# constantinpape/torch-em

Hardware: AMD Instinct MI355X
Metric: voxels/sec fwd+bwd, UNet3d 1x128^3 bs=2 (higher is better)
Workload: dtype f32-class (forward convs on normalised activations: fp32 operands split into 2 fp16 terms = 22 mantissa bits, lo plane scaled by 2^12 with its own fp32 accumulator, 3 fp16 MFMAs per product; other forward convs 3 bf16 terms / 6 MFMAs; data-gradient convs 2 bf16 terms / 3 MFMAs (16-bit products); WEI

## Files before the change

torch_em_amd/csrc/capi.hip:

```cpp
#include "tem_common.h"
#include "conv_internal.h"
#include "tem_act.h"
#include <stdarg.h>
#include <string.h>

static thread_local char g_err[512] = "";

void tem_set_error(const char* fmt, ...) {
    va_list ap;
    va_start(ap, fmt);
    vsnprintf(g_err, sizeof(g_err), fmt, ap);
    va_end(ap);
}

extern "C" const char* tem_last_error(void) { return g_err; }

struct TemOption {
    const char* name;
    long long def;
};
static const TemOption g_opt_table[TEM_OPT_COUNT] = {
    {"wgrad_zs", 3},
    {"wgrad_zs_persist", 1},
    {"wgrad_sums", 1},
    {"wgrad_sums_min_mb", 128},
    {"fwd_persistent", -1},
    {"conv_fwd_variant", -1},
    {"conv1x1_stream", 1},
    {"fwd_ksplit_chunks", 0},
    {"wgrad_cus", 256},
    {"upsample_generic", 0},
    {"team_min_units", 0},
    {"zr_splitk", 1},
    {"zr_wide", 1},
    {"zr_tile_blocks", 1},
    {"dice_vox", 1},
    {"upsample2_ch8", 1},
    {"pool_vec8", 2},
    {"fp32_zr", 1},
};
static long long g_opt_val[TEM_OPT_COUNT];
static bool g_opt_set[TEM_OPT_COUNT];

long long tem_option(int id) {
    if (id < 0 || id >= TEM_OPT_COUNT) return 0;
    return __atomic_load_n(&g_opt_set[id], __ATOMIC_RELAXED) ? __atomic_load_n(&g_opt_val[id], __ATOMIC_RELAXED)
                                                            : g_opt_table[id].def;
}
static int opt_find(const char* name) {
    if (!name) return -1;
    for (int i = 0; i < TEM_OPT_COUNT; ++i)
        if (!strcmp(name, g_opt_table[i].name)) return i;
    return -1;
}
extern "C" int tem_set_option(const char* name, int64_t value) {
    const int id = opt_find(name);
    TEM_REQUIRE(id >= 0, "tem_set_option: unknown option '%s'", name ? name : "(null)");
    __atomic_store_n(&g_opt_val[id], (long long)value, __ATOMIC_RELAXED);
    __atomic_store_n(&g_opt_set[id], true, __ATOMIC_RELAXED);
    return TEM_OK;
}
extern "C" int tem_get_option(const char* name, int64_t* value) {
    const int id = opt_find(name);
    TEM_REQUIRE(id >= 0 && value, "tem_get_option: unknown option '%s'", name ? name : "(null)");
    *value = (int64_t)tem_option(id);
    return TEM_OK;
}
extern "C" int tem_version(void) { return 100; }

extern "C" int tem_device_cus(void) {
    int dev = 0;
    if (hipGetDevice(&dev) != hipSuccess) return TEM_ELAUNCH;
    hipDeviceProp_t prop;
    if (hipGetDeviceProperties(&prop, dev) != hipSuccess) return TEM_ELAUNCH;
    return prop.multiProcessorCount;
}

#define TT_V 64
#define TT_C 32

__global__ __launch_bounds__(256) void k_nchw_to_nhwc(const float* __restrict__ src, float* __restrict__ dst,
                                                      int64_t dst_ld, int C, int64_t V, int64_t vtiles, int ctiles) {
    __shared__ float tile[TT_C][TT_V + 1];
    int64_t ntiles = vtiles * ctiles;
    int n = blockIdx.y;
    for (int64_t t = blockIdx.x; t < ntiles; t += gridDim.x) {
        int ct = (int)(t % ctiles);
        int64_t vt = t / ctiles;
        int64_t v0 = vt * TT_V;
        int c0 = ct * TT_C;
        for (int i = threadIdx.x; i < TT_C * TT_V; i += 256) {
            int c = i / TT_V, v = i % TT_V;
            float val = 0.f;
            if (c0 + c < C && v0 + v < V) val = src[((int64_t)n * C + c0 + c) * V + v0 + v];
            tile[c][v] = val;
        }
        __syncthreads();
        for (int i = threadIdx.x; i < TT_C * TT_V; i += 256) {
            int v = i / TT_C, c = i % TT_C;
            if (c0 + c < C && v0 + v < V) dst[((int64_t)n * V + v0 + v) * dst_ld + c0 + c] = tile[c][v];
        }
        __syncthreads();
    }
}

__global__ __launch_bounds__(256) void k_nhwc_to_nchw(const float* __restrict__ src, int64_t src_ld,
                                                      float* __restrict__ dst, int C, int64_t V, int64_t vtiles,
                                                      int ctiles) {
    __shared__ float tile[TT_C][TT_V + 1];
    int64_t ntiles = vtiles * ctiles;
    int n = blockIdx.y;
    for (int64_t t = blockIdx.x; t < ntiles; t += gridDim.x) {
        int ct = (int)(t % ctiles);
        int64_t vt = t / ctiles;
        int64_t v0 = vt * TT_V;
        int c0 = ct * TT_C;
        for (int i = threadIdx.x; i < TT_C * TT_V; i += 256) {
            int v = i / TT_C, c = i % TT_C;
            float val = 0.f;
            if (c0 + c < C && v0 + v < V) val = src[((int64_t)n * V + v0 + v) * src_ld + c0 + c];
            tile[c][v] = val;
        }
        __syncthreads();
        for (int i = threadIdx.x; i < TT_C * TT_V; i += 256) {
            int c = i / TT_V, v = i % TT_V;
            if (c0 + c < C && v0 + v < V) dst[((int64_t)n * C + c0 + c) * V + v0 + v] = tile[c][v];
        }
        __syncthreads();
    }
}

extern "C" int tem_nchw_to_nhwc(const float* src, float* dst, int64_t dst_ld, int N, int C, int64_t V,
                                tem_stream_t stream) {
    TEM_REQUIRE(src && dst && N > 0 && C > 0 && V > 0 && dst_ld >= C, "tem_nchw_to_nhwc: bad arguments");
    int64_t vtiles = tem_cdiv(V, TT_V);
    int ctiles = (int)tem_cdiv(C, TT_C);
    int64_t nt = vtiles * ctiles;
    dim3 grid((unsigned)(nt > 4096 ? 4096 : nt), N);
    hipLaunchKernelGGL(k_nchw_to_nhwc, grid, dim3(256), 0, (hipStream_t)stream, src, dst, dst_ld, C, V, vtiles, ctiles);
    TEM_CHECK_LAUNCH("tem_nchw_to_nhwc");
    return TEM_OK;
}

extern "C" int tem_nhwc_to_nchw(const float* src, int64_t src_ld, float* dst, int N, int C, int64_t V,
                                tem_stream_t stream) {
    TEM_REQUIRE(src && dst && N > 0 && C > 0 && V > 0 && src_ld >= C, "tem_nhwc_to_nchw: bad arguments");
    int64_t vtiles = tem_cdiv(V, TT_V);
    int ctiles = (int)tem_cdiv(C, TT_C);
    int64_t nt = vtiles * ctiles;
    dim3 grid((unsigned)(nt > 4096 ? 4096 : nt), N);
    hipLaunchKernelGGL(k_nhwc_to_nchw, grid, dim3(256), 0, (hipStream_t)stream, src, src_ld, dst, C, V, vtiles, ctiles);
    TEM_CHECK_LAUNCH("tem_nhwc_to_nchw");
    return TEM_OK;
}

#define STD_BLOCKS 256

__global__ __launch_bounds__(256) void k_std_partial(const float* __restrict__ x, int64_t L, double* __restrict__ part) {
    int n = blockIdx.y;
    const float* row = x + (int64_t)n * L;
    double s = 0.0, ss = 0.0;
    for (int64_t i = (int64_t)blockIdx.x * 256 + threadIdx.x; i < L; i += (int64_t)gridDim.x * 256) {
        double v = (double)row[i];
        s += v;
        ss += v * v;
    }
    s = tem_wave_sum_d(s);
    ss = tem_wave_sum_d(ss);
    __shared__ double sh[2][4];
    int w = threadIdx.x >> 6;
    if ((threadIdx.x & 63) == 0) { sh[0][w] = s; sh[1][w] = ss; }
    __syncthreads();
    if (threadIdx.x == 0) {
        part[((int64_t)n * gridDim.x + blockIdx.x) * 2 + 0] = sh[0][0] + sh[0][1] + sh[0][2] + sh[0][3];
        part[((int64_t)n * gridDim.x + blockIdx.x) * 2 + 1] = sh[1][0] + sh[1][1] + sh[1][2] + sh[1][3];
    }
}

__global__ __launch_bounds__(256) void k_std_apply(const float* __restrict__ x, float* __restrict__ y, int64_t L,
                                                   const double* __restrict__ part, int nblk, float eps) {
    int n = blockIdx.y;
    __shared__ float sh_mean, sh_inv;
    if (threadIdx.x == 0) {
        double s = 0.0, ss = 0.0;
        for (int b = 0; b < nblk; ++b) {
            s += part[((int64_t)n * nblk + b) * 2 + 0];
            ss += part[((int64_t)n * nblk + b) * 2 + 1];
        }
        double mean = s / (double)L;
        double var = ss / (double)L - mean * mean;
        if (var < 0.0) var = 0.0;
        sh_mean = (float)mean;
        sh_inv = (float)(1.0 / (sqrt(var) + (double)eps));
    }
    __syncthreads();
    float mean = sh_mean, inv = sh_inv;
    const float* row = x + (int64_t)n * L;
    float* out = y + (int64_t)n * L;
    for (int64_t i = (int64_t)blockIdx.x * 256 + threadIdx.x; i < L; i += (int64_t)gridDim.x * 256)
        out[i] = (row[i] - mean) * inv;
}

extern "C" int tem_standardize(const float* x, float* y, int N, int64_t L, float eps, void* ws, int64_t ws_bytes,
                               tem_stream_t stream) {
    TEM_REQUIRE(x && y && ws && N > 0 && L > 0, "tem_standardize: bad arguments");
    int nblk = (int)(tem_cdiv(L, 256) < STD_BLOCKS ? tem_cdiv(L, 256) : STD_BLOCKS);
    if ((int64_t)N * nblk * 2 * (int64_t)sizeof(double) > ws_bytes) {
        tem_set_error("tem_standardize: workspace too small (%lld bytes needed)",
                      (long long)((int64_t)N * nblk * 2 * sizeof(double)));
        return TEM_EWS;
    }
    hipLaunchKernelGGL(k_std_partial, dim3(nblk, N), dim3(256), 0, (hipStream_t)stream, x, L, (double*)ws);
    hipLaunchKernelGGL(k_std_apply, dim3(nblk, N), dim3(256), 0, (hipStream_t)stream, x, y, L, (const double*)ws, nblk, eps);
    TEM_CHECK_LAUNCH("tem_standardize");
    return TEM_OK;
}

__global__ __launch_bounds__(256) void k_act_bwd(const float* __restrict__ gy, const float* __restrict__ y,
                                                 float* __restrict__ gx, int64_t n, int act) {
    for (int64_t i = (int64_t)blockIdx.x * 256 + threadIdx.x; i < n; i += (int64_t)gridDim.x * 256) {
        float yv = y[i], g = gy[i];
        gx[i] = (act == TEM_ACT_SIGMOID) ? g * yv * (1.f - yv) : ((yv > 0.f) ? g : 0.f);
    }
}

extern "C" int tem_act_bwd(const float* gy, const float* y, float* gx, int64_t n, int act, tem_stream_t stream) {
    TEM_REQUIRE(gy && y && gx && n > 0, "tem_act_bwd: bad arguments");
    TEM_REQUIRE(act == TEM_ACT_RELU || act == TEM_ACT_SIGMOID, "tem_act_bwd: Invalid activation: %d", act);
    hipLaunchKernelGGL(k_act_bwd, dim3(tem_grid_1d(n, 256)), dim3(256), 0, (hipStream_t)stream, gy, y, gx, n, act);
    TEM_CHECK_LAUNCH("tem_act_bwd");
    return TEM_OK;
}
```

torch_em_amd/csrc/pool_upsample.hip:

```cpp
#include "tem_common.h"
#include "tem_act.h"

template <int VEC>
struct VecT;
template <>
struct VecT<4> {
    typedef float4 type;
};
template <>
struct VecT<1> {
    typedef float type;
};

#ifndef TEM_POOL_NT
#define TEM_POOL_NT 0
#endif
template <int VEC, typename T>
__device__ __forceinline__ void ld_vec(const T* p, float (&v)[VEC]) {
    if constexpr (VEC == 8) {
        act_ld8(p, v);
    } else if constexpr (VEC == 4) {
        const float4 t = act_ld4(p);
        v[0] = t.x; v[1] = t.y; v[2] = t.z; v[3] = t.w;
    } else {
// ... 562 lines not shown
                }
            ++cnt;
        }
    }
    return cnt;
}

__device__ __forceinline__ void utu_axis(int i, int f, int in, float (&a)[3], float& s) {
    a[0] = a[1] = a[2] = 0.f;
    s = 0.f;
    const int olo = max(0, f * i - f), ohi = min(in * f - 1, f * i + 2 * f - 1);
    for (int o = olo; o <= ohi; ++o) {
        const float w = lin_w(o, f, in, i);
        if (w == 0.f) continue;
        s += w;
#pragma unroll
        for (int d = -1; d <= 1; ++d)
            if (i + d >= 0 && i + d < in) a[d + 1] = fmaf(w, lin_w(o, f, in, i + d), a[d + 1]);
    }
}

template <int VEC, typename T>
__global__ __launch_bounds__(256) void k_upsample_bwd(const T* __restrict__ gy, int64_t gy_ld,
                                                      T* __restrict__ gx, int64_t gx_ld, int D, int H, int W, int C,
                                                      int fz, int fy, int fx, const T* __restrict__ u, int64_t u_ld,
                                                      const float* __restrict__ ncoef, int64_t ncoef_ld) {
    const int Do = D * fz, Ho = H * fy, Wo = W * fx;
    const int cq = C / VEC;
    int row = blockIdx.x;
    const int yi = row % H;
    row /= H;
    const int zi = row % D;
    const int n = row / D;
    const int zlo = max(0, fz * zi - fz), zhi = min(Do - 1, fz * zi + 2 * fz - 1);
    const int ylo = max(0, fy * yi - fy), yhi = min(Ho - 1, fy * yi + 2 * fy - 1);
    const bool fast = fz <= 2 && fy <= 2 && fx <= 2;
    int zidx[4], yidx[4];
    float zw[4], yw[4];
    int nzt = 0;
    if (fast) {
        nzt = upb_taps(zlo, zhi, fz, D, zi, zidx, zw);
        upb_taps(ylo, yhi, fy, H, yi, yidx, yw);
    }
    float az[3] = {0.f, 0.f, 0.f}, ay[3] = {0.f, 0.f, 0.f}, sz = 0.f, sy = 0.f;
    if (ncoef) {
        utu_axis(zi, fz, D, az, sz);
        utu_axis(yi, fy, H, ay, sy);
    }
    for (int i = threadIdx.x; i < W * cq; i += 256) {
        const int xi = i / cq, c0 = (i % cq) * VEC;
        const int xlo = max(0, fx * xi - fx), xhi = min(Wo - 1, fx * xi + 2 * fx - 1);
        float acc[VEC];
#pragma unroll
        for (int j = 0; j < VEC; ++j) acc[j] = 0.f;
        if (fast) {
            int xidx[4];
            float xw[4];
            upb_taps(xlo, xhi, fx, W, xi, xidx, xw);
            for (int kz = 0; kz < nzt; ++kz) {
                const int64_t rz = ((int64_t)n * Do + zidx[kz]) * Ho;
                float t[4][4][VEC];
#pragma unroll
                for (int ky = 0; ky < 4; ++ky)
#pragma unroll
                    for (int kx = 0; kx < 4; ++kx) ld_vec<VEC>(gy + ((rz + yidx[ky]) * Wo + xidx[kx]) * gy_ld + c0, t[ky][kx]);
#pragma unroll
                for (int ky = 0; ky < 4; ++ky)
#pragma unroll
                    for (int kx = 0; kx < 4; ++kx) {
                        const float w = zw[kz] * yw[ky] * xw[kx];
#pragma unroll
                        for (int j = 0; j < VEC; ++j) acc[j] = fmaf(w, t[ky][kx][j], acc[j]);
                    }
            }
        } else
        for (int zo = zlo; zo <= zhi; ++zo) {
            float wz = lin_w(zo, fz, D, zi);
            if (wz == 0.f) continue;
            for (int yo = ylo; yo <= yhi; ++yo) {
                float wy = lin_w(yo, fy, H, yi);
                if (wy == 0.f) continue;
                const int64_t r = (((int64_t)n * Do + zo) * Ho + yo) * Wo;
                for (int xo = xlo; xo <= xhi; ++xo) {
                    float wx = lin_w(xo, fx, W, xi);
                    if (wx == 0.f) continue;
                    float t[VEC];
                    ld_vec<VEC>(gy + (r + xo) * gy_ld + c0, t);
                    const float w = wz * wy * wx;
#pragma unroll
                    for (int j = 0; j < VEC; ++j) acc[j] = fmaf(w, t[j], acc[j]);
                }
            }
        }
        int64_t v = (((int64_t)n * D + zi) * H + yi) * W + xi;
        if (ncoef) {
            float ax[3], sx;
            utu_axis(xi, fx, W, ax, sx);
            const float S = sz * sy * sx;
            float q[VEC];
#pragma unroll
            for (int j = 0; j < VEC; ++j) q[j] = 0.f;
#pragma unroll
            for (int dz = -1; dz <= 1; ++dz) {
                const int zc = min(max(zi + dz, 0), D - 1);
                float t[3][3][VEC];
#pragma unroll
                for (int dy = -1; dy <= 1; ++dy) {
                    const int yc = min(max(yi + dy, 0), H - 1);
#pragma unroll
                    for (int dx = -1; dx <= 1; ++dx) {
                        const int xc = min(max(xi + dx, 0), W - 1);
                        ld_vec<VEC>(u + ((((int64_t)n * D + zc) * H + yc) * W + xc) * u_ld + c0, t[dy + 1][dx + 1]);
                    }
                }
#pragma unroll
                for (int dy = -1; dy <= 1; ++dy)
#pragma unroll
                    for (int dx = -1; dx <= 1; ++dx) {
                        const float wq = az[dz + 1] * ay[dy + 1] * ax[dx + 1];
#pragma unroll
                        for (int j = 0; j < VEC; ++j) q[j] = fmaf(wq, t[dy + 1][dx + 1][j], q[j]);
                    }
            }
#pragma unroll
            for (int j = 0; j < VEC; ++j) {
                const float4 kc = *reinterpret_cast<const float4*>(ncoef + (int64_t)n * ncoef_ld + (c0 + j) * 4);
                acc[j] = kc.x * acc[j] - kc.y * S - kc.z * (q[j] - kc.w * S);
            }
        }
        st_vec<VEC>(gx + v * gx_ld + c0, acc);
    }
}

template <int CH>
struct FV {
    float v[CH];
};
template <int CH, typename T>
__device__ __forceinline__ FV<CH> ldv(const T* p) {
    FV<CH> r;
    if constexpr (CH == 8) {
        act_ld8(p, r.v);
    } else {
        const float4 t = act_ld4(p);
        r.v[0] = t.x; r.v[1] = t.y; r.v[2] = t.z; r.v[3] = t.w;
    }
    return r;
}
template <int CH, typename T>
__device__ __forceinline__ void stv(T* p, const FV<CH>& a) {
    if constexpr (CH == 8) act_st8(p, a.v);
    else act_st4(p, make_float4(a.v[0], a.v[1], a.v[2], a.v[3]));
}
template <int CH>
__device__ __forceinline__ FV<CH> fv_zero() {
    FV<CH> r;
#pragma unroll
    for (int j = 0; j < CH; ++j) r.v[j] = 0.f;
    return r;
}
template <int CH>
__device__ __forceinline__ FV<CH> lerp2(float l0, const FV<CH>& a, float l1, const FV<CH>& b) {
    FV<CH> r;
#pragma unroll
    for (int j = 0; j < CH; ++j) r.v[j] = l0 * a.v[j] + l1 * b.v[j];
    return r;
}

template <int FZ, typename T, int CH = 4>
__global__ __launch_bounds__(256) void k_upsample2_fwd(const T* __restrict__ x, int64_t x_ld, T* __restrict__ y,
                                                       int64_t y_ld, int D, int H, int W, int C,
                                                       float* __restrict__ part) {
    extern __shared__ float lsu[];
    const int Ho = 2 * H, Wo = 2 * W;
    const int cq = C / CH;
    int row = blockIdx.x;
    const int yi = row % H;
    row /= H;
    const int zi = row % D;
    const int n = row / D;
    const int ym = max(yi - 1, 0), yp = min(yi + 1, H - 1);
    const int zm = max(zi - 1, 0), zp = min(zi + 1, D - 1);
    const float ya0 = yi == 0 ? 1.f : 0.25f, ya1 = yi == 0 ? 0.f : 0.75f;
    const float za0 = zi == 0 ? 1.f : 0.25f, za1 = zi == 0 ? 0.f : 0.75f;
    const int zrow[3] = {zm, zi, zp}, yrow[3] = {ym, yi, yp};
    float s1[CH], s2[CH];
#pragma unroll
    for (int j = 0; j < CH; ++j) s1[j] = s2[j] = 0.f;
    for (int i = threadIdx.x; i < W * cq; i += 256) {
        const int xi = i / cq, c0 = (i % cq) * CH;
        const int xm = max(xi - 1, 0), xp = min(xi + 1, W - 1);
        const float xa0 = xi == 0 ? 1.f : 0.25f, xa1 = xi == 0 ? 0.f : 0.75f;
        FV<CH> Y[FZ == 2 ? 3 : 1][2][2];
#pragma unroll
        for (int kz = 0; kz < (FZ == 2 ? 3 : 1); ++kz) {
            const int zc = FZ == 2 ? zrow[kz] : zi;
            FV<CH> X[3][2];
#pragma unroll
            for (int ky = 0; ky < 3; ++ky) {
                const T* r = x + ((((int64_t)n * D + zc) * H + yrow[ky]) * W) * x_ld + c0;
                const FV<CH> a = ldv<CH>(r + (int64_t)xm * x_ld), b = ldv<CH>(r + (int64_t)xi * x_ld), c = ldv<CH>(r + (int64_t)xp * x_ld);
                X[ky][0] = lerp2(xa0, a, xa1, b);
                X[ky][1] = lerp2(0.75f, b, 0.25f, c);
            }
#pragma unroll
            for (int sx = 0; sx < 2; ++sx) {
                Y[kz][0][sx] = lerp2(ya0, X[0][sx], ya1, X[1][sx]);
                Y[kz][1][sx] = lerp2(0.75f, X[1][sx], 0.25f, X[2][sx]);
            }
            __builtin_amdgcn_sched_barrier(0);
        }
#pragma unroll
        for (int sz = 0; sz < FZ; ++sz)
#pragma unroll
            for (int sy = 0; sy < 2; ++sy)
#pragma unroll
                for (int sx = 0; sx < 2; ++sx) {
                    FV<CH> o;
                    if constexpr (FZ == 2)
                        o = sz == 0 ? lerp2(za0, Y[0][sy][sx], za1, Y[1][sy][sx]) : lerp2(0.75f, Y[1][sy][sx], 0.25f, Y[2][sy][sx]);
                    else
                        o = Y[0][sy][sx];
                    const int64_t vo = (((int64_t)n * (D * FZ) + zi * FZ + sz) * Ho + 2 * yi + sy) * Wo + 2 * xi + sx;
                    if constexpr (sizeof(T) == 2) {
#pragma unroll
                        for (int j = 0; j < CH; j += 2) {
                            const unsigned pk = act_pk<T>(o.v[j], o.v[j + 1]);
                            o.v[j] = act_lo<T>(pk);
                            o.v[j + 1] = act_hi<T>(pk);
                        }
                    }
                    stv<CH>(y + vo * y_ld + c0, o);
#pragma unroll
                    for (int j = 0; j < CH; ++j) {
                        s1[j] += o.v[j];
                        s2[j] = fmaf(o.v[j], o.v[j], s2[j]);
                    }
                }
    }
    if (part) {
        const int wv = threadIdx.x >> 6, lane = threadIdx.x & 63;
#pragma unroll
        for (int j = 0; j < CH; ++j) {
            for (int o = cq; o < 64; o <<= 1) {
                s1[j] += __shfl_xor(s1[j], o, 64);
                s2[j] += __shfl_xor(s2[j], o, 64);
            }
            if (lane < cq) {
                lsu[(wv * C + lane * CH + j) * 2 + 0] = s1[j];
                lsu[(wv * C + lane * CH + j) * 2 + 1] = s2[j];
            }
        }
        __syncthreads();
        for (int t = threadIdx.x; t < 2 * C; t += 256) {
            float a = 0.f;
            for (int w4 = 0; w4 < 4; ++w4) a += lsu[w4 * 2 * C + t];
            part[((int64_t)n * D * H + (int64_t)zi * H + yi) * 2 * C + t] = a;
        }
    }
}

struct UpbAxis {
    int idx[6];
    float w[2][4];
};
__device__ __forceinline__ UpbAxis upb_axis2(int i0, int in) {
    UpbAxis a;
    const int out = 2 * in;
#pragma unroll
    for (int k = 0; k < 6; ++k) a.idx[k] = min(max(2 * i0 - 1 + k, 0), out - 1);
#pragma unroll
    for (int c = 0; c < 2; ++c)
#pragma unroll
        for (int k = 0; k < 4; ++k) {
            const int o = 2 * i0 - 1 + 2 * c + k;
            a.w[c][k] = (o >= 0 && o < out && i0 + c < in) ? lin_w(o, 2, in, i0 + c) : 0.f;
        }
    return a;
}
__device__ __forceinline__ float upb_w(int o, int in, int i) {
    return (o >= 0 && o < 2 * in && i < in) ? lin_w(o, 2, in, i) : 0.f;
}
__device__ __forceinline__ float pick3(const float (&a)[3], int d) {
    return d == 0 ? a[0] : d == 1 ? a[1] : d == 2 ? a[2] : 0.f;
}
struct UtuAxis {
    int idx[4];
    float a[2][3];
    float s[2];
};
__device__ __forceinline__ UtuAxis utu_axis2(int i0, int f, int in) {
    UtuAxis r;
#pragma unroll
    for (int k = 0; k < 4; ++k) r.idx[k] = min(max(i0 - 1 + k, 0), in - 1);
#pragma unroll
    for (int c = 0; c < 2; ++c) {
        r.a[c][0] = r.a[c][1] = r.a[c][2] = 0.f;
        r.s[c] = 0.f;
        if (i0 + c < in) utu_axis(i0 + c, f, in, r.a[c], r.s[c]);
    }
    return r;
}

template <int FZ, typename T, int CH = 4>
__global__ __launch_bounds__(256) void k_upsample2_bwd(const T* __restrict__ gy, int64_t gy_ld,
                                                       T* __restrict__ gx, int64_t gx_ld, int D, int H, int W, int C,
                                                       const T* __restrict__ u, int64_t u_ld,
                                                       const float* __restrict__ ncoef, int64_t ncoef_ld) {
    constexpr int CZ = FZ == 2 ? 2 : 1;
    constexpr int NZF = FZ == 2 ? 6 : 1;
    const int Do = D * FZ, Ho = 2 * H, Wo = 2 * W;
    const int cq = C / CH;
    const int Hp = (H + 1) >> 1, Wp = (W + 1) >> 1, Dp = (D + CZ - 1) / CZ;
    int row = blockIdx.x;
    const int y0 = (row % Hp) * 2;
    row /= Hp;
    const int z0 = (row % Dp) * CZ;
    const int n = row / Dp;
    for (int i = threadIdx.x; i < Wp * cq; i += 256) {
        const int x0 = (i / cq) * 2, c0 = (i % cq) * CH;
        const UpbAxis ax = upb_axis2(x0, W);
        FV<CH> acc[CZ][2][2];
#pragma unroll
        for (int a = 0; a < CZ; ++a)
#pragma unroll
            for (int b = 0; b < 2; ++b)
#pragma unroll
                for (int c = 0; c < 2; ++c) acc[a][b][c] = fv_zero<CH>();
#pragma unroll 1
        for (int kz = 0; kz < NZF; ++kz) {
            const int oz = FZ == 2 ? 2 * z0 - 1 + kz : z0;
            const int zf = min(max(oz, 0), Do - 1);
            float wz[CZ];
#pragma unroll
            for (int a = 0; a < CZ; ++a) wz[a] = FZ == 2 ? upb_w(oz, D, z0 + a) : 1.f;
            FV<CH> pp[2][2];
#pragma unroll
            for (int b = 0; b < 2; ++b)
#pragma unroll
                for (int c = 0; c < 2; ++c) pp[b][c] = fv_zero<CH>();
#pragma unroll 2
            for (int ky = 0; ky < 6; ++ky) {
                const int oy = 2 * y0 - 1 + ky;
                const float wy[2] = {upb_w(oy, H, y0), upb_w(oy, H, y0 + 1)};
                const T* r = gy + ((((int64_t)n * Do + zf) * Ho + min(max(oy, 0), Ho - 1)) * Wo) * gy_ld + c0;
                FV<CH> t[6];
#pragma unroll
                for (int kx = 0; kx < 6; ++kx) t[kx] = ldv<CH>(r + (int64_t)ax.idx[kx] * gy_ld);
#pragma unroll
                for (int c = 0; c < 2; ++c)
#pragma unroll
                    for (int j = 0; j < CH; ++j) {
                        const float xr = ax.w[c][0] * t[2 * c].v[j] + ax.w[c][1] * t[2 * c + 1].v[j] +
                                         ax.w[c][2] * t[2 * c + 2].v[j] + ax.w[c][3] * t[2 * c + 3].v[j];
                        pp[0][c].v[j] = fmaf(wy[0], xr, pp[0][c].v[j]);
                        pp[1][c].v[j] = fmaf(wy[1], xr, pp[1][c].v[j]);
                    }
            }
#pragma unroll
            for (int a = 0; a < CZ; ++a)
#pragma unroll
                for (int b = 0; b < 2; ++b)
#pragma unroll
                    for (int c = 0; c < 2; ++c)
#pragma unroll
                        for (int j = 0; j < CH; ++j) acc[a][b][c].v[j] = fmaf(wz[a], pp[b][c].v[j], acc[a][b][c].v[j]);
        }
        if (ncoef) {
            const UtuAxis bx = utu_axis2(x0, 2, W), by = utu_axis2(y0, 2, H), bz = utu_axis2(z0, FZ, D);
            FV<CH> q[CZ][2][2];
#pragma unroll
            for (int a = 0; a < CZ; ++a)
#pragma unroll
                for (int b = 0; b < 2; ++b)
#pragma unroll
                    for (int c = 0; c < 2; ++c) q[a][b][c] = fv_zero<CH>();
            constexpr int NZU = FZ == 2 ? 4 : 1;
#pragma unroll 1
            for (int kz = 0; kz < NZU; ++kz) {
                const int zc = FZ == 2 ? min(max(z0 - 1 + kz, 0), D - 1) : z0;
                float wz[CZ];
#pragma unroll
                for (int a = 0; a < CZ; ++a) wz[a] = FZ == 2 ? pick3(bz.a[a], kz - a) : 1.f;
                FV<CH> qp[2][2];
#pragma unroll
                for (int b = 0; b < 2; ++b)
#pragma unroll
                    for (int c = 0; c < 2; ++c) qp[b][c] = fv_zero<CH>();
#pragma unroll 2
                for (int ky = 0; ky < 4; ++ky) {
                    const float wy[2] = {pick3(by.a[0], ky), pick3(by.a[1], ky - 1)};
                    const T* r = u + ((((int64_t)n * D + zc) * H + min(max(y0 - 1 + ky, 0), H - 1)) * W) * u_ld + c0;
                    FV<CH> t[4];
#pragma unroll
                    for (int kx = 0; kx < 4; ++kx) t[kx] = ldv<CH>(r + (int64_t)bx.idx[kx] * u_ld);
#pragma unroll
                    for (int c = 0; c < 2; ++c)
#pragma unroll
                        for (int j = 0; j < CH; ++j) {
                            const float xr = bx.a[c][0] * t[c].v[j] + bx.a[c][1] * t[c + 1].v[j] + bx.a[c][2] * t[c + 2].v[j];
                            qp[0][c].v[j] = fmaf(wy[0], xr, qp[0][c].v[j]);
                            qp[1][c].v[j] = fmaf(wy[1], xr, qp[1][c].v[j]);
                        }
                }
#pragma unroll
                for (int a = 0; a < CZ; ++a)
#pragma unroll
                    for (int b = 0; b < 2; ++b)
#pragma unroll
                        for (int c = 0; c < 2; ++c)
#pragma unroll
                            for (int j = 0; j < CH; ++j) q[a][b][c].v[j] = fmaf(wz[a], qp[b][c].v[j], q[a][b][c].v[j]);
            }
            float4 kc[CH];
#pragma unroll
            for (int j = 0; j < CH; ++j) kc[j] = *reinterpret_cast<const float4*>(ncoef + (int64_t)n * ncoef_ld + (c0 + j) * 4);
#pragma unroll
            for (int a = 0; a < CZ; ++a)
#pragma unroll
                for (int b = 0; b < 2; ++b)
#pragma unroll
                    for (int c = 0; c < 2; ++c) {
                        const float S = (FZ == 2 ? bz.s[a] : 1.f) * by.s[b] * bx.s[c];
#pragma unroll
                        for (int j = 0; j < CH; ++j)
                            acc[a][b][c].v[j] = kc[j].x * acc[a][b][c].v[j] - kc[j].y * S - kc[j].z * (q[a][b][c].v[j] - kc[j].w * S);
                    }
        }
#pragma unroll
        for (int a = 0; a < CZ; ++a)
#pragma unroll
            for (int b = 0; b < 2; ++b)
#pragma unroll
                for (int c = 0; c < 2; ++c) {
                    if (z0 + a >= D || y0 + b >= H || x0 + c >= W) continue;
                    const int64_t v = (((int64_t)n * D + z0 + a) * H + y0 + b) * W + x0 + c;
                    stv<CH>(gx + v * gx_ld + c0, acc[a][b][c]);
                }
    }
}

template <int VEC, typename T>
__global__ __launch_bounds__(256) void k_upsample_stats(const T* __restrict__ u, int64_t u_ld, int D, int H, int W,
                                                        int C, int fz, int fy, int fx, float* __restrict__ part) {
    extern __shared__ float lsu[];
    const int cq = C / VEC;
    int row = blockIdx.x;
    const int yi = row % H;
    row /= H;
    const int zi = row % D;
    const int n = row / D;
    float az[3], ay[3], sz, sy;
    utu_axis(zi, fz, D, az, sz);
    utu_axis(yi, fy, H, ay, sy);
    float s1[VEC], s2[VEC];
#pragma unroll
    for (int j = 0; j < VEC; ++j) s1[j] = s2[j] = 0.f;
    for (int i = threadIdx.x; i < W * cq; i += 256) {
        const int xi = i / cq, c0 = (i % cq) * VEC;
        float ax[3], sx;
        utu_axis(xi, fx, W, ax, sx);
        const float S = sz * sy * sx;
        float q[VEC], uc[VEC];
#pragma unroll
        for (int j = 0; j < VEC; ++j) q[j] = 0.f;
        ld_vec<VEC>(u + ((((int64_t)n * D + zi) * H + yi) * W + xi) * u_ld + c0, uc);
#pragma unroll
        for (int dz = -1; dz <= 1; ++dz) {
            const int zc = min(max(zi + dz, 0), D - 1);
            float t[3][3][VEC];
#pragma unroll
            for (int dy = -1; dy <= 1; ++dy) {
                const int yc = min(max(yi + dy, 0), H - 1);
#pragma unroll
                for (int dx = -1; dx <= 1; ++dx) {
                    const int xc = min(max(xi + dx, 0), W - 1);
                    ld_vec<VEC>(u + ((((int64_t)n * D + zc) * H + yc) * W + xc) * u_ld + c0, t[dy + 1][dx + 1]);
                }
            }
#pragma unroll
            for (int dy = -1; dy <= 1; ++dy)
#pragma unroll
                for (int dx = -1; dx <= 1; ++dx) {
                    const float wq = az[dz + 1] * ay[dy + 1] * ax[dx + 1];
#pragma unroll
                    for (int j = 0; j < VEC; ++j) q[j] = fmaf(wq, t[dy + 1][dx + 1][j], q[j]);
                }
        }
#pragma unroll
        for (int j = 0; j < VEC; ++j) {
            s1[j] = fmaf(S, uc[j], s1[j]);
            s2[j] = fmaf(uc[j], q[j], s2[j]);
        }
    }
    const int wv = threadIdx.x >> 6, lane = threadIdx.x & 63;
#pragma unroll
    for (int j = 0; j < VEC; ++j) {
        for (int o = cq; o < 64; o <<= 1) {
            s1[j] += __shfl_xor(s1[j], o, 64);
            s2[j] += __shfl_xor(s2[j], o, 64);
        }
        if (lane < cq) {
            lsu[(wv * C + lane * VEC + j) * 2 + 0] = s1[j];
            lsu[(wv * C + lane * VEC + j) * 2 + 1] = s2[j];
        }
    }
    __syncthreads();
    for (int t = threadIdx.x; t < 2 * C; t += 256) {
        float a = 0.f;
        for (int w4 = 0; w4 < 4; ++w4) a += lsu[w4 * 2 * C + t];
        part[((int64_t)n * D * H + (int64_t)zi * H + yi) * 2 * C + t] = a;
    }
}

static int upsample_stats_impl(const void* u, int64_t u_ld, int N, int D, int H, int W, int C, int fz, int fy, int fx,
                               float* part, int st, tem_stream_t stream) {
    TEM_REQUIRE(u && part && N > 0 && C > 0 && u_ld >= C && D > 0 && H > 0 && W > 0 && fz > 0 && fy > 0 && fx > 0,
                "tem_upsample_stats: bad arguments");
    TEM_REQUIRE(st >= 0 && st <= 2, "tem_upsample_stats: unknown storage type %d", st);
    const int cq = C / 4;
    TEM_REQUIRE(C % 4 == 0 && cq <= 64 && (cq & (cq - 1)) == 0 && u_ld % 4 == 0 && ((uintptr_t)u % tem_st_align4(st) == 0),
                "tem_upsample_stats: needs C = 4 * 2^k <= 256 channels, rows aligned to 4 elements (got C=%d)", C);
    int64_t rows = (int64_t)N * D * H;
    TEM_REQUIRE(rows < (1ll << 31), "tem_upsample_stats: too many rows");
    TEM_ST_SWITCH(st, T, hipLaunchKernelGGL((k_upsample_stats<4, T>), dim3((unsigned)rows), dim3(256), (size_t)4 * C * 2 * sizeof(float),
                                            (hipStream_t)stream, (const T*)u, u_ld, D, H, W, C, fz, fy, fx, part));
    TEM_CHECK_LAUNCH("tem_upsample_stats");
    return TEM_OK;
}
extern "C" int tem_upsample_stats(const float* u, int64_t u_ld, int N, int D, int H, int W, int C, int fz, int fy, int fx,
                                  float* part, tem_stream_t stream) {
    return upsample_stats_impl(u, u_ld, N, D, H, W, C, fz, fy, fx, part, 0, stream);
}
extern "C" int tem_upsample_stats_st(const void* u, int64_t u_ld, int N, int D, int H, int W, int C, int fz, int fy, int fx,
                                     float* part, int st, tem_stream_t stream) {
    return upsample_stats_impl(u, u_ld, N, D, H, W, C, fz, fy, fx, part, st, stream);
}

static inline bool upsample2_ok(int C, int fz, int fy, int fx) {
    return fy == 2 && fx == 2 && (fz == 1 || fz == 2) && C % 4 == 0 && !tem_option(TEM_OPT_UPSAMPLE_GENERIC);
}

extern "C" int tem_upsample_fwd_stats_ok(int C, int fz, int fy, int fx) {
    const int cq = C / 4;
    return upsample2_ok(C, fz, fy, fx) && cq <= 64 && (cq & (cq - 1)) == 0;
}

static int upsample_fwd_impl(const void* x, int64_t x_ld, void* y, int64_t y_ld, int N, int D, int H, int W, int C, int fz,
                             int fy, int fx, float* part, int st, tem_stream_t stream) {
    TEM_REQUIRE(x && y && N > 0 && C > 0 && x_ld >= C && y_ld >= C && D > 0 && H > 0 && W > 0,
                "tem_upsample_fwd: bad arguments");
    TEM_REQUIRE(st >= 0 && st <= 2, "tem_upsample_fwd: unknown storage type %d", st);
    TEM_REQUIRE(fz > 0 && fy > 0 && fx > 0, "tem_upsample_fwd: bad factors");
    const bool v4 = vec4_ok(C, {x, y}, {x_ld, y_ld}, st);
    TEM_REQUIRE(!part || (tem_upsample_fwd_stats_ok(C, fz, fy, fx) && v4),
                "tem_upsample_fwd_stats: needs factors (1|2, 2, 2), C = 4 * 2^k <= 256 and rows aligned to 4 elements");
    int64_t rows = (int64_t)N * D * fz * H * fy;
    TEM_REQUIRE(rows < (1ll << 31), "tem_upsample_fwd: too many rows");
    const size_t ldsb = part ? (size_t)4 * C * 2 * sizeof(float) : 0;
    if (fz == 1 && upsample2_ok(C, fz, fy, fx) && vec8_ok(C, {x, y}, {x_ld, y_ld}, st) && ((C / 8) & (C / 8 - 1)) == 0 && C / 8 <= 64) {
        const int64_t crow = (int64_t)N * D * H;
        TEM_ST16_SWITCH(st, T, {
            hipLaunchKernelGGL((k_upsample2_fwd<1, T, 8>), dim3((unsigned)crow), dim3(256), ldsb, (hipStream_t)stream, (const T*)x,
                               x_ld, (T*)y, y_ld, D, H, W, C, part);
        });
        TEM_CHECK_LAUNCH("tem_upsample_fwd");
        return TEM_OK;
    }
    TEM_ST_SWITCH(st, T, {
        const T* xs = (const T*)x;
        T* ys = (T*)y;
        if (upsample2_ok(C, fz, fy, fx) && v4) {
            const int64_t crow = (int64_t)N * D * H;
            if (fz == 2)
                hipLaunchKernelGGL((k_upsample2_fwd<2, T>), dim3((unsigned)crow), dim3(256), ldsb, (hipStream_t)stream, xs, x_ld, ys,
                                   y_ld, D, H, W, C, part);
            else
                hipLaunchKernelGGL((k_upsample2_fwd<1, T>), dim3((unsigned)crow), dim3(256), ldsb, (hipStream_t)stream, xs, x_ld, ys,
                                   y_ld, D, H, W, C, part);
        } else if (v4)
            hipLaunchKernelGGL((k_upsample_fwd<4, T>), dim3((unsigned)rows), dim3(256), 0, (hipStream_t)stream, xs, x_ld, ys,
                               y_ld, D, H, W, C, fz, fy, fx);
        else
            hipLaunchKernelGGL((k_upsample_fwd<1, T>), dim3((unsigned)rows), dim3(256), 0, (hipStream_t)stream, xs, x_ld, ys,
                               y_ld, D, H, W, C, fz, fy, fx);
    });
    TEM_CHECK_LAUNCH("tem_upsample_fwd");
    return TEM_OK;
}

extern "C" int tem_upsample_fwd_stats(const float* x, int64_t x_ld, float* y, int64_t y_ld, int N, int D, int H, int W,
                                      int C, int fz, int fy, int fx, float* part, tem_stream_t stream) {
    TEM_REQUIRE(part, "tem_upsample_fwd_stats: bad arguments");
    return upsample_fwd_impl(x, x_ld, y, y_ld, N, D, H, W, C, fz, fy, fx, part, 0, stream);
}

extern "C" int tem_upsample_fwd(const float* x, int64_t x_ld, float* y, int64_t y_ld, int N, int D, int H, int W, int C,
                                int fz, int fy, int fx, tem_stream_t stream) {
    return upsample_fwd_impl(x, x_ld, y, y_ld, N, D, H, W, C, fz, fy, fx, nullptr, 0, stream);
}

extern "C" int tem_upsample_fwd_st(const void* x, int64_t x_ld, void* y, int64_t y_ld, int N, int D, int H, int W, int C,
                                   int fz, int fy, int fx, float* part, int st, tem_stream_t stream) {
    return upsample_fwd_impl(x, x_ld, y, y_ld, N, D, H, W, C, fz, fy, fx, part, st, stream);
}

static int upsample_bwd_impl(const void* gy, int64_t gy_ld, void* gx, int64_t gx_ld, int N, int D, int H, int W,
                             int C, int fz, int fy, int fx, const void* u, int64_t u_ld, const float* ncoef,
                             int64_t ncoef_ld, int st, tem_stream_t stream) {
    TEM_REQUIRE(gy && gx && N > 0 && C > 0 && gy_ld >= C && gx_ld >= C && D > 0 && H > 0 && W > 0,
                "tem_upsample_bwd: bad arguments");
    TEM_REQUIRE(st >= 0 && st <= 2, "tem_upsample_bwd: unknown storage type %d", st);
    TEM_REQUIRE(fz > 0 && fy > 0 && fx > 0, "tem_upsample_bwd: bad factors");
    int64_t rows = (int64_t)N * D * H;
    TEM_REQUIRE(rows < (1ll << 31), "tem_upsample_bwd: too many rows");
    const int64_t pairs = (int64_t)N * ((D + fz - 1) / fz) * ((H + 1) / 2) * ((W + 1) / 2) * (C / 4);
    if (upsample2_ok(C, fz, fy, fx) && pairs >= 2 * 65536 && vec8_ok(C, {gy, gx, u}, {gy_ld, gx_ld, u ? u_ld : 0}, st) && tem_option(TEM_OPT_UPSAMPLE2_CH8)) {
        TEM_ST16_SWITCH(st, T, {
            if (fz == 2) {
                const int64_t prow = (int64_t)N * ((D + 1) / 2) * ((H + 1) / 2);
                hipLaunchKernelGGL((k_upsample2_bwd<2, T, 8>), dim3((unsigned)prow), dim3(256), 0, (hipStream_t)stream, (const T*)gy,
                                   gy_ld, (T*)gx, gx_ld, D, H, W, C, (const T*)u, u_ld, ncoef, ncoef_ld);
            } else {
                const int64_t prow = (int64_t)N * D * ((H + 1) / 2);
                hipLaunchKernelGGL((k_upsample2_bwd<1, T, 8>), dim3((unsigned)prow), dim3(256), 0, (hipStream_t)stream, (const T*)gy,
                                   gy_ld, (T*)gx, gx_ld, D, H, W, C, (const T*)u, u_ld, ncoef, ncoef_ld);
            }
        });
        TEM_CHECK_LAUNCH("tem_upsample_bwd");
        return TEM_OK;
    }
    TEM_ST_SWITCH(st, T, {
        const T* gys = (const T*)gy;
        const T* us = (const T*)u;
        T* gxs = (T*)gx;
        if (upsample2_ok(C, fz, fy, fx) && pairs >= 65536 && vec4_ok(C, {gy, gx, u}, {gy_ld, gx_ld, u_ld}, st)) {
            if (fz == 2) {
                const int64_t prow = (int64_t)N * ((D + 1) / 2) * ((H + 1) / 2);
                hipLaunchKernelGGL((k_upsample2_bwd<2, T>), dim3((unsigned)prow), dim3(256), 0, (hipStream_t)stream, gys, gy_ld, gxs,
                                   gx_ld, D, H, W, C, us, u_ld, ncoef, ncoef_ld);
            } else {
                const int64_t prow = (int64_t)N * D * ((H + 1) / 2);
                hipLaunchKernelGGL((k_upsample2_bwd<1, T>), dim3((unsigned)prow), dim3(256), 0, (hipStream_t)stream, gys, gy_ld, gxs,
                                   gx_ld, D, H, W, C, us, u_ld, ncoef, ncoef_ld);
            }
        } else if (vec4_ok(C, {gy, gx, u}, {gy_ld, gx_ld, u ? u_ld : 0}, st))
            hipLaunchKernelGGL((k_upsample_bwd<4, T>), dim3((unsigned)rows), dim3(256), 0, (hipStream_t)stream, gys, gy_ld, gxs,
                               gx_ld, D, H, W, C, fz, fy, fx, us, u_ld, ncoef, ncoef_ld);
        else
            hipLaunchKernelGGL((k_upsample_bwd<1, T>), dim3((unsigned)rows), dim3(256), 0, (hipStream_t)stream, gys, gy_ld, gxs,
                               gx_ld, D, H, W, C, fz, fy, fx, us, u_ld, ncoef, ncoef_ld);
    });
    TEM_CHECK_LAUNCH("tem_upsample_bwd");
    return TEM_OK;
}

extern "C" int tem_upsample_bwd(const float* gy, int64_t gy_ld, float* gx, int64_t gx_ld, int N, int D, int H, int W,
                                int C, int fz, int fy, int fx, tem_stream_t stream) {
    return upsample_bwd_impl(gy, gy_ld, gx, gx_ld, N, D, H, W, C, fz, fy, fx, nullptr, 0, nullptr, 0, 0, stream);
}

extern "C" int tem_upsample_bwd_norm(const float* gy, int64_t gy_ld, float* gx, int64_t gx_ld, int N, int D, int H,
                                     int W, int C, int fz, int fy, int fx, const float* u, int64_t u_ld,
                                     const float* ncoef, int64_t ncoef_ld, tem_stream_t stream) {
    TEM_REQUIRE(u && ncoef, "tem_upsample_bwd_norm: bad arguments");
    return tem_upsample_bwd_st(gy, gy_ld, gx, gx_ld, N, D, H, W, C, fz, fy, fx, u, u_ld, ncoef, ncoef_ld, TEM_ST_F32, stream);
}

extern "C" int tem_upsample_bwd_st(const void* gy, int64_t gy_ld, void* gx, int64_t gx_ld, int N, int D, int H, int W, int C,
                                   int fz, int fy, int fx, const void* u, int64_t u_ld, const float* ncoef, int64_t ncoef_ld,
                                   int st, tem_stream_t stream) {
    TEM_REQUIRE((u == nullptr) == (ncoef == nullptr), "tem_upsample_bwd_norm: u and ncoef come together");
    if (ncoef) {
        TEM_REQUIRE(u_ld >= C && ncoef_ld >= 4 * C && ((uintptr_t)ncoef % 16 == 0) && ncoef_ld % 4 == 0,
                    "tem_upsample_bwd_norm: bad arguments");
        TEM_REQUIRE(st >= 0 && st <= 2 && (C % 4 || (u_ld % 4 == 0 && (uintptr_t)u % tem_st_align4(st) == 0)),
                    "tem_upsample_bwd_norm: u must be aligned to 4 elements");
    }
    return upsample_bwd_impl(gy, gy_ld, gx, gx_ld, N, D, H, W, C, fz, fy, fx, u, u_ld, ncoef, ncoef_ld, st, stream);
}
```

torch_em_amd/csrc/tem_common.h:

```cpp
#pragma once
#include <hip/hip_runtime.h>
#include <stdint.h>
#include <stdio.h>
#include "../../include/tem_hip.h"

void tem_set_error(const char* fmt, ...);

enum {
    TEM_OPT_WGRAD_ZS = 0,
    TEM_OPT_WGRAD_ZS_PERSIST,
    TEM_OPT_WGRAD_SUMS,
    TEM_OPT_WGRAD_SUMS_MIN_MB,
    TEM_OPT_FWD_PERSISTENT,
    TEM_OPT_CONV_FWD_VARIANT,
    TEM_OPT_CONV1X1_STREAM,
    TEM_OPT_FWD_KSPLIT_CHUNKS,
    TEM_OPT_WGRAD_CUS,
    TEM_OPT_UPSAMPLE_GENERIC,
    TEM_OPT_TEAM_MIN_UNITS,
    TEM_OPT_ZR_SPLITK,
    TEM_OPT_ZR_WIDE,
    TEM_OPT_ZR_TILE_BLOCKS,
    TEM_OPT_DICE_VOX,
    TEM_OPT_UPSAMPLE2_CH8,
    TEM_OPT_POOL_VEC8,
    TEM_OPT_FP32_ZR,
    TEM_OPT_COUNT
};
long long tem_option(int id);

#define TEM_REQUIRE(cond, ...)                 \
    do {                                       \
        if (!(cond)) {                         \
            tem_set_error(__VA_ARGS__);        \
            return TEM_EINVAL;                 \
        }                                      \
    } while (0)

#define TEM_TRY(call)                          \
    do {                                       \
        const int rc__ = (call);               \
        if (rc__ != TEM_OK) return rc__;       \
    } while (0)

#define TEM_CHECK_LAUNCH(name)                                                   \
    do {                                                                         \
        hipError_t e__ = hipGetLastError();                                      \
        if (e__ != hipSuccess) {                                                 \
            tem_set_error("%s: launch failed: %s", name, hipGetErrorString(e__)); \
            return TEM_ELAUNCH;                                                  \
        }                                                                        \
    } while (0)

static inline int64_t tem_cdiv(int64_t a, int64_t b) { return (a + b - 1) / b; }
static inline int64_t tem_align_up(int64_t a, int64_t b) { return tem_cdiv(a, b) * b; }

static inline int tem_grid_1d(int64_t work_items, int block, int max_blocks = 256 * 8) {
    int64_t g = tem_cdiv(work_items, block);
    if (g > max_blocks) g = max_blocks;
    if (g < 1) g = 1;
    return (int)g;
}

#define TEM_WAVE 64

__device__ __forceinline__ float tem_amax4(float m, float a, float b, float c, float d) {
    return __builtin_fmaxf(__builtin_fmaxf(m, __builtin_fmaxf(__builtin_fabsf(a), __builtin_fabsf(b))),
                           __builtin_fmaxf(__builtin_fabsf(c), __builtin_fabsf(d)));
}
__device__ __forceinline__ void tem_amax_commit(unsigned* amax, float m) {
    unsigned u = __builtin_bit_cast(unsigned, m);
#pragma unroll
    for (int o = 32; o > 0; o >>= 1) u = max(u, (unsigned)__shfl_xor((int)u, o, 64));
    if ((threadIdx.x & 63) == 0 && u > __atomic_load_n(amax, __ATOMIC_RELAXED)) atomicMax(amax, u);
}

__device__ __forceinline__ float tem_wave_sum(float v) {
#pragma unroll
    for (int o = 32; o > 0; o >>= 1) v += __shfl_xor(v, o, 64);
    return v;
}
__device__ __forceinline__ double tem_wave_sum_d(double v) {
#pragma unroll
    for (int o = 32; o > 0; o >>= 1) v += __shfl_xor(v, o, 64);
    return v;
}

__device__ __forceinline__ int tem_xcd_remap(int bid, int nwg) {
    const int nx = 8;
    int q = nwg / nx, r = nwg % nx;
    int xcd = bid % nx, idx = bid / nx;
    int base = (xcd < r) ? xcd * (q + 1) : r * (q + 1) + (xcd - r) * q;
    return base + idx;
}
```

Measured before the change: 280.3 million.

## March upsample-backward blocks along z to reuse shared gradient planes

The trilinear upsample backward kernel can now have each block walk a chunk of consecutive z-pairs. The last two output planes of one pair are accumulated into the next pair's accumulator, so those planes are not re-read and re-filtered. Blocks are also remapped across XCDs. The chunk size is picked so the grid keeps at least 512 blocks. The cost is more registers from the extra accumulator set and fewer blocks.

```diff
diff --git a/torch_em_amd/csrc/capi.hip b/torch_em_amd/csrc/capi.hip
--- a/torch_em_amd/csrc/capi.hip
+++ b/torch_em_amd/csrc/capi.hip
@@ -38,6 +38,7 @@
     {"upsample2_ch8", 1},
     {"pool_vec8", 2},
     {"fp32_zr", 1},
+    {"upsample2_bwd_march", 1},
 };
 static long long g_opt_val[TEM_OPT_COUNT];
 static bool g_opt_set[TEM_OPT_COUNT];
diff --git a/torch_em_amd/csrc/pool_upsample.hip b/torch_em_amd/csrc/pool_upsample.hip
--- a/torch_em_amd/csrc/pool_upsample.hip
+++ b/torch_em_amd/csrc/pool_upsample.hip
@@ -888,33 +888,40 @@
     return r;
 }
 
-template <int FZ, typename T, int CH = 4>
+template <int FZ, typename T, int CH = 4, int MODE = 0>
 __global__ __launch_bounds__(256) void k_upsample2_bwd(const T* __restrict__ gy, int64_t gy_ld,
                                                        T* __restrict__ gx, int64_t gx_ld, int D, int H, int W, int C,
                                                        const T* __restrict__ u, int64_t u_ld,
-                                                       const float* __restrict__ ncoef, int64_t ncoef_ld) {
+                                                       const float* __restrict__ ncoef, int64_t ncoef_ld, int zc) {
+    constexpr bool MARCH = MODE == 2;
+    static_assert(!MARCH || FZ == 2, "only factor 2 in z has planes that two pairs share");
     constexpr int CZ = FZ == 2 ? 2 : 1;
     constexpr int NZF = FZ == 2 ? 6 : 1;
     const int Do = D * FZ, Ho = 2 * H, Wo = 2 * W;
     const int cq = C / CH;
     const int Hp = (H + 1) >> 1, Wp = (W + 1) >> 1, Dp = (D + CZ - 1) / CZ;
-    int row = blockIdx.x;
+    const int nch = MARCH ? (Dp + zc - 1) / zc : Dp;
+    int row = MODE ? tem_xcd_remap(blockIdx.x, gridDim.x) : blockIdx.x;
     const int y0 = (row % Hp) * 2;
     row /= Hp;
-    const int z0 = (row % Dp) * CZ;
-    const int n = row / Dp;
+    const int zbeg = (row % nch) * (MARCH ? zc : 1) * CZ;
+    const int zend = MARCH ? min(zbeg + zc * CZ, Dp * CZ) : zbeg + CZ;
+    const int n = row / nch;
     for (int i = threadIdx.x; i < Wp * cq; i += 256) {
         const int x0 = (i / cq) * 2, c0 = (i % cq) * CH;
         const UpbAxis ax = upb_axis2(x0, W);
-        FV<CH> acc[CZ][2][2];
+        FV<CH> acc[CZ][2][2], nxt[CZ][2][2];
 #pragma unroll
         for (int a = 0; a < CZ; ++a)
 #pragma unroll
             for (int b = 0; b < 2; ++b)
 #pragma unroll
-                for (int c = 0; c < 2; ++c) acc[a][b][c] = fv_zero<CH>();
+                for (int c = 0; c < 2; ++c) acc[a][b][c] = nxt[a][b][c] = fv_zero<CH>();
+        int z0 = zbeg, kz0 = 0;
 #pragma unroll 1
-        for (int kz = 0; kz < NZF; ++kz) {
+        do {
+#pragma unroll 1
+        for (int kz = kz0; kz < NZF; ++kz) {
             const int oz = FZ == 2 ? 2 * z0 - 1 + kz : z0;
             const int zf = min(max(oz, 0), Do - 1);
             float wz[CZ];
@@ -951,6 +958,20 @@
                     for (int c = 0; c < 2; ++c)
 #pragma unroll
                         for (int j = 0; j < CH; ++j) acc[a][b][c].v[j] = fmaf(wz[a], pp[b][c].v[j], acc[a][b][c].v[j]);
+            if constexpr (MARCH) {
+                if (kz >= 4) {
+#pragma unroll
+                    for (int a = 0; a < CZ; ++a) {
+                        const float wn = upb_w(oz, D, z0 + CZ + a);
+#pragma unroll
+                        for (int b = 0; b < 2; ++b)
+#pragma unroll
+                            for (int c = 0; c < 2; ++c)
+#pragma unroll
+                                for (int j = 0; j < CH; ++j) nxt[a][b][c].v[j] = fmaf(wn, pp[b][c].v[j], nxt[a][b][c].v[j]);
+                    }
+                }
+            }
         }
         if (ncoef) {
             const UtuAxis bx = utu_axis2(x0, 2, W), by = utu_axis2(y0, 2, H), bz = utu_axis2(z0, FZ, D);
@@ -1023,6 +1044,20 @@
                     const int64_t v = (((int64_t)n * D + z0 + a) * H + y0 + b) * W + x0 + c;
                     stv<CH>(gx + v * gx_ld + c0, acc[a][b][c]);
                 }
+        if constexpr (MARCH) {
+#pragma unroll
+            for (int a = 0; a < CZ; ++a)
+#pragma unroll
+                for (int b = 0; b < 2; ++b)
+#pragma unroll
+                    for (int c = 0; c < 2; ++c) {
+                        acc[a][b][c] = nxt[a][b][c];
+                        nxt[a][b][c] = fv_zero<CH>();
+                    }
+            kz0 = 2;
+        }
+        z0 += CZ;
+        } while (MARCH && z0 < zend);
     }
 }
 
@@ -1191,6 +1226,36 @@
     return upsample_fwd_impl(x, x_ld, y, y_ld, N, D, H, W, C, fz, fy, fx, part, st, stream);
 }
 
+#define UPB_MARCH_MIN_BLOCKS 512
+static int upsample2_bwd_zc(int64_t columns, int Dp, int ch) {
+    const long long opt = tem_option(TEM_OPT_UPSAMPLE2_BWD_MARCH);
+    if (opt != 1) return opt < 0 ? 0 : (int)(opt < Dp ? opt : Dp);
+    for (int zc = ch == 8 ? 1 : 8; zc > 1; zc >>= 1)
+        if (columns * tem_cdiv(Dp, zc) >= UPB_MARCH_MIN_BLOCKS) return zc;
+    return 1;
+}
+
+template <typename T, int CH>
+static void launch_upsample2_bwd(const T* gy, int64_t gy_ld, T* gx, int64_t gx_ld, int N, int D, int H, int W, int C, int fz,
+                                 const T* u, int64_t u_ld, const float* ncoef, int64_t ncoef_ld, hipStream_t stream) {
+    const int Dp = fz == 2 ? (D + 1) / 2 : D;
+    const int64_t columns = (int64_t)N * ((H + 1) / 2);
+    const int zc = fz == 2 ? upsample2_bwd_zc(columns, Dp, CH) : (tem_option(TEM_OPT_UPSAMPLE2_BWD_MARCH) != 0);
+    const dim3 grid((unsigned)(columns * (zc > 1 ? tem_cdiv(Dp, zc) : Dp)));
+#define UPB_LAUNCH(FZ, MODE) \
+    hipLaunchKernelGGL((k_upsample2_bwd<FZ, T, CH, MODE>), grid, dim3(256), 0, stream, gy, gy_ld, gx, gx_ld, D, H, W, C, u, u_ld, \
+                       ncoef, ncoef_ld, zc)
+    if (fz == 2) {
+        if (zc > 1) UPB_LAUNCH(2, 2);
+        else if (zc == 1) UPB_LAUNCH(2, 1);
+        else UPB_LAUNCH(2, 0);
+    } else {
+        if (zc) UPB_LAUNCH(1, 1);
+        else UPB_LAUNCH(1, 0);
+    }
+#undef UPB_LAUNCH
+}
+
 static int upsample_bwd_impl(const void* gy, int64_t gy_ld, void* gx, int64_t gx_ld, int N, int D, int H, int W,
                              int C, int fz, int fy, int fx, const void* u, int64_t u_ld, const float* ncoef,
                              int64_t ncoef_ld, int st, tem_stream_t stream) {
@@ -1203,15 +1268,8 @@
     const int64_t pairs = (int64_t)N * ((D + fz - 1) / fz) * ((H + 1) / 2) * ((W + 1) / 2) * (C / 4);
     if (upsample2_ok(C, fz, fy, fx) && pairs >= 2 * 65536 && vec8_ok(C, {gy, gx, u}, {gy_ld, gx_ld, u ? u_ld : 0}, st) && tem_option(TEM_OPT_UPSAMPLE2_CH8)) {
         TEM_ST16_SWITCH(st, T, {
-            if (fz == 2) {
-                const int64_t prow = (int64_t)N * ((D + 1) / 2) * ((H + 1) / 2);
-                hipLaunchKernelGGL((k_upsample2_bwd<2, T, 8>), dim3((unsigned)prow), dim3(256), 0, (hipStream_t)stream, (const T*)gy,
-                                   gy_ld, (T*)gx, gx_ld, D, H, W, C, (const T*)u, u_ld, ncoef, ncoef_ld);
-            } else {
-                const int64_t prow = (int64_t)N * D * ((H + 1) / 2);
-                hipLaunchKernelGGL((k_upsample2_bwd<1, T, 8>), dim3((unsigned)prow), dim3(256), 0, (hipStream_t)stream, (const T*)gy,
-                                   gy_ld, (T*)gx, gx_ld, D, H, W, C, (const T*)u, u_ld, ncoef, ncoef_ld);
-            }
+            launch_upsample2_bwd<T, 8>((const T*)gy, gy_ld, (T*)gx, gx_ld, N, D, H, W, C, fz, (const T*)u, u_ld, ncoef, ncoef_ld,
+                                       (hipStream_t)stream);
         });
         TEM_CHECK_LAUNCH("tem_upsample_bwd");
         return TEM_OK;
@@ -1221,15 +1279,7 @@
         const T* us = (const T*)u;
         T* gxs = (T*)gx;
         if (upsample2_ok(C, fz, fy, fx) && pairs >= 65536 && vec4_ok(C, {gy, gx, u}, {gy_ld, gx_ld, u_ld}, st)) {
-            if (fz == 2) {
-                const int64_t prow = (int64_t)N * ((D + 1) / 2) * ((H + 1) / 2);
-                hipLaunchKernelGGL((k_upsample2_bwd<2, T>), dim3((unsigned)prow), dim3(256), 0, (hipStream_t)stream, gys, gy_ld, gxs,
-                                   gx_ld, D, H, W, C, us, u_ld, ncoef, ncoef_ld);
-            } else {
-                const int64_t prow = (int64_t)N * D * ((H + 1) / 2);
-                hipLaunchKernelGGL((k_upsample2_bwd<1, T>), dim3((unsigned)prow), dim3(256), 0, (hipStream_t)stream, gys, gy_ld, gxs,
-                                   gx_ld, D, H, W, C, us, u_ld, ncoef, ncoef_ld);
-            }
+            launch_upsample2_bwd<T, 4>(gys, gy_ld, gxs, gx_ld, N, D, H, W, C, fz, us, u_ld, ncoef, ncoef_ld, (hipStream_t)stream);
         } else if (vec4_ok(C, {gy, gx, u}, {gy_ld, gx_ld, u ? u_ld : 0}, st))
             hipLaunchKernelGGL((k_upsample_bwd<4, T>), dim3((unsigned)rows), dim3(256), 0, (hipStream_t)stream, gys, gy_ld, gxs,
                                gx_ld, D, H, W, C, fz, fy, fx, us, u_ld, ncoef, ncoef_ld);
diff --git a/torch_em_amd/csrc/tem_common.h b/torch_em_amd/csrc/tem_common.h
--- a/torch_em_amd/csrc/tem_common.h
+++ b/torch_em_amd/csrc/tem_common.h
@@ -25,6 +25,7 @@
     TEM_OPT_UPSAMPLE2_CH8,
     TEM_OPT_POOL_VEC8,
     TEM_OPT_FP32_ZR,
+    TEM_OPT_UPSAMPLE2_BWD_MARCH,
     TEM_OPT_COUNT
 };
 long long tem_option(int id);
```

After: 281.3 million (median of 6 runs). No clear change (+0.4%).
